# WonderfulToolchain/psxavenc

Measured on AMD Instinct MI355X. Metric: bs_v2_320x240_frames_per_sec, higher is better.
Workload: dtype int32

## Files before the change

psxavenc_amd/csrc/mdec_kernels.hip:

```cpp

#include <hip/hip_runtime.h>
#include <stdint.h>
#include <type_traits>
#include <stdlib.h>
#include <string.h>

#include "bs_vlc_lut.h"
#include "mdec_search.h"
#include "psxhip_internal.h"
#include "wave_ops.h"

namespace {

constexpr int kWavesSmall = 12, kOccSmall = 6;
constexpr int kWavesLarge = 16, kOccLarge = 4;
constexpr int kTileStride = 72;
constexpr int kZStride = 64;
constexpr int kPilotMax = 4;
constexpr int kMaxTiles = 16;
constexpr uint32_t kNoMb = 0xFFFFu;
constexpr uint32_t kRetryEmpty = 0xFFFFFFFFu, kRetryAbandoned = 0xFFFFFFFEu;
constexpr int kQueueWord = 64;
constexpr int kStartedWord = 96;
constexpr int kLeaveWord = 8;
constexpr int kLeaveWrongShift = 32, kLeaveTriedShift = 48;
constexpr unsigned kTrustCap = 63u;
constexpr float kCkMargin = 1000.0f;
constexpr int kNoTicket = 0x7FFFFFFF;
constexpr int kPilotWord = 10;
constexpr int kDistrustWord = 4;
constexpr int kQueueReservedShift = 32, kQueueHeadShift = 48;
constexpr unsigned kQueueMask = 0xFFFFu;
template <typename T>
__device__ __forceinline__ T queue_peek(T* p, int looks) {
    return looks < 4096 ? __hip_atomic_load(p, __ATOMIC_RELAXED, __HIP_MEMORY_SCOPE_AGENT) : atomicOr(p, (T)0);
}

__constant__ uint16_t c_ac_len16[BS_LUT_SIZE];
__constant__ uint32_t c_ac_code[BS_LUT_SIZE];
__constant__ uint8_t c_zagzig[64];
__constant__ uint8_t c_quant_zz[64];
__constant__ uint8_t c_dc_prefix[2][8];
// ... 11 lines not shown
    int first[kMaxBatches];
    int n_batches;
    size_t frame_stride;
    int width, height, nx, ny, nmb;
    int n_frames;
    int n_tickets;
    int uniform_max_size;
    size_t out_stride;
    int out_words;
    int out_tile;
    int max_frame_size;
    int stg_words;
    int trips;
    int it_step;
    const uint32_t* order;
    unsigned int* ticket;
    unsigned int* hint;
    unsigned int* retry;
    int retry_patience;
    int retry_cap;
    int trust_mode;
    unsigned long long* stats;
    uint32_t col_k[16];
};
typedef const BatchDesc __attribute__((address_space(4))) * BatchPtr;
typedef const int __attribute__((address_space(4))) * FirstPtr;
#define PSX_BATCHES_MANY() (((FirstPtr)(batch_table() + kMaxBatches))[kMaxBatches] > 1)
__device__ __forceinline__ BatchPtr batch_table() {
    BatchPtr p = (BatchPtr)__builtin_amdgcn_kernarg_segment_ptr();
    asm volatile("" : "+s"(p));
    return p;
}
#define PSX_JOB_INT(member) (((FirstPtr)((const char __attribute__((address_space(4)))*)batch_table() + offsetof(FrameJob, member)))[0])
__device__ __forceinline__ unsigned int* retry_slots(const FrameJob& job) {
    unsigned int* p = job.retry;
    asm volatile("" : "+s"(p));
    return p;
}
__device__ __forceinline__ unsigned long long* queue_state(const FrameJob& job) { return (unsigned long long*)&job.ticket[kQueueWord]; }
__device__ __forceinline__ unsigned draw_ticket(const FrameJob& job) { return (unsigned)atomicAdd(queue_state(job), 1ull); }
__device__ __forceinline__ unsigned long long* leave_word(const FrameJob& job) { return (unsigned long long*)&job.ticket[kLeaveWord]; }
enum {
    S_DC_BITS = 0,
    S_STG_NEXT,
    S_FOREIGN,
    S_CNT_F,
// ... 265 lines not shown

__host__ __device__ constexpr size_t lds_fixed_bytes(int waves) {
    size_t b = 0;
    b += (size_t)S_COUNT * 4;
    b += BS_LUT_SIZE * 2;
    b = (b + 3) & ~(size_t)3;
    b += BS_LUT_SIZE * 4;
    b += 32;
    b = (b + 15) & ~(size_t)15;
    b += 2 * 64 * 16 + 2 * 64;
    b += (size_t)waves * kWaveTileBytes;
    return (b + 15) & ~(size_t)15;
}
__host__ __device__ inline size_t lds_bytes(int nmb, int out_words, int stg_words, int waves) {
    size_t b = lds_fixed_bytes(waves);
    b += (size_t)out_words * 4;
    b += (size_t)stg_words * 4;
    b += (size_t)nmb * 4;
    b += (size_t)nmb * 4;
    b += (size_t)dc_chunks(nmb) * 16;
    b += (size_t)nmb * 6 * 2;
    return (b + 15) & ~(size_t)15;
}
template <int WAVES>
__device__ __forceinline__ Lds carve(char* base, int nmb, int out_words, int stg_words) {
    Lds L;
    size_t b = 0;
    L.scalars = (int*)(base + b);         b += (size_t)S_COUNT * 4;
    L.ac_len16 = (uint16_t*)(base + b);   b += BS_LUT_SIZE * 2;                    b = (b + 3) & ~(size_t)3;
    L.ac_code = (uint32_t*)(base + b);    b += BS_LUT_SIZE * 4;
    L.dc_plen = (uint8_t*)(base + b);     b += 16;
    L.dc_prefix = (uint8_t*)(base + b);   b += 16;                                 b = (b + 15) & ~(size_t)15;
    L.tab_sel = (uint4*)(base + b);       b += 64 * 16;
    L.tab_pix = (uint4*)(base + b);       b += 64 * 16;
    L.tab_nat = (uint8_t*)(base + b);     b += 64;
    L.qzz = (uint8_t*)(base + b);         b += 64;
    L.tiles = (int16_t*)(base + b);       b += (size_t)WAVES * kWaveTileBytes;     b = (b + 15) & ~(size_t)15;
    L.out = (uint32_t*)(base + b);        b += (size_t)out_words * 4;
    L.stg = (uint32_t*)(base + b);        b += (size_t)stg_words * 4;
    L.rec = (uint32_t*)(base + b);        b += (size_t)nmb * 4;
    L.mb_off = (uint32_t*)(base + b);     b += (size_t)nmb * 4;
    L.dc_fn = (int*)(base + b);           b += (size_t)dc_chunks(nmb) * 16;
    L.dcv = (int16_t*)(base + b);
    return L;
}

// ... 128 lines not shown
}
template <int CTRL>
__device__ __forceinline__ StepFn dpp_stepfn(const StepFn& f) {
    StepFn e;
    e.thr = __builtin_amdgcn_update_dpp(f.thr, f.thr, CTRL, 0xF, 0xF, false);
    e.lo = __builtin_amdgcn_update_dpp(f.lo, f.lo, CTRL, 0xF, 0xF, false);
    e.hi = __builtin_amdgcn_update_dpp(f.hi, f.hi, CTRL, 0xF, 0xF, false);
    return e;
}
__device__ __forceinline__ void scan_stepfn(StepFn& f, int lane) {
    StepFn e;
    e = dpp_stepfn<0x111>(f); if ((lane & 15) >= 1) f = compose(e, f);
    e = dpp_stepfn<0x112>(f); if ((lane & 15) >= 2) f = compose(e, f);
    e = dpp_stepfn<0x114>(f); if ((lane & 15) >= 4) f = compose(e, f);
    e = dpp_stepfn<0x118>(f); if ((lane & 15) >= 8) f = compose(e, f);
    e = dpp_stepfn<0x142>(f); if (lane & 16) f = compose(e, f);
    e = dpp_stepfn<0x143>(f); if (lane >= 32) f = compose(e, f);
}

template <int CODEC, int WAVES, int OCC, bool STATS>
__global__ __launch_bounds__(WAVES * 64, OCC) void mdec_encode_frames_kernel(const FrameJob job) {
    constexpr int kWavesPerGroup = WAVES;
    constexpr int kThreads = WAVES * 64;
    extern __shared__ __attribute__((aligned(16))) char smem[];
    const Lds L = carve<WAVES>(smem, job.nmb, job.out_words, job.stg_words);

    const int tid = (int)threadIdx.x;
    unsigned long long t_entry = 0, t_first = 0;
    if (STATS) t_entry = wall_clock64();
    const int wid = __builtin_amdgcn_readfirstlane(tid >> 6);
    const int nmb = job.nmb, nx = job.nx, ny = job.ny, W = job.width, H = job.height;
    const int nblk = nmb * 6;
    constexpr int kPilotPerWave = 2;
    const int pilot_rounds = (WAVES == kWavesLarge || nmb >= 600) ? 2 : 1;
    const int n_pilot = nmb < kWavesPerGroup * pilot_rounds ? nmb : kWavesPerGroup * pilot_rounds;

    constexpr int kLutTrips = (BS_LUT_SIZE + kThreads - 1) / kThreads;
    uint16_t lut_len[kLutTrips];
    uint32_t lut_code[kLutTrips];
#pragma unroll
    for (int j = 0; j < kLutTrips; j++) {
        const int i = tid + j * kThreads;
        lut_len[j] = i < BS_LUT_SIZE ? c_ac_len16[i] : (uint16_t)0;
        lut_code[j] = i < BS_LUT_SIZE ? c_ac_code[i] : 0u;
    }
    const uint8_t pro_plen = c_dc_plen[(tid >> 3) & 1][tid & 7], pro_prefix = c_dc_prefix[(tid >> 3) & 1][tid & 7];
// ... 350 lines not shown
                bits = wave::reduce_add(bits);
                if (lane == 0 && bits) atomicAdd(&L.scalars[S_DC_BITS], bits);
            }
            group_sync(1);
        }
        mark(1);
        const int dc_bits = CODEC == 0 ? 10 * nblk : L.scalars[S_DC_BITS];
        const int fixed_bits = dc_bits + 2 * nblk + 10;

        float cf[6];
        uint2 plo = make_uint2(0, 0), phi = make_uint2(0, 0);

        auto fetch_at = [&](uint32_t row, uint32_t col) {
            const uint4 tp = L.tab_pix[lane];
            const uint32_t o_lo = tp.x + (row << tp.z) + col, o_hi = o_lo + tp.y;
            plo = *(const uint2*)(frame + o_lo);
            phi = *(const uint2*)(frame + o_hi);
        };
        auto fetch = [&](int fx, int fy) { fetch_at((uint32_t)fy * (uint32_t)(8 * W), (uint32_t)fx * 16u); };
        auto mb_bytes = [&](const uint4& ts, uint32_t& b_lo, uint32_t& b_hi) {
            b_lo = __builtin_amdgcn_perm(plo.y, plo.x, ts.x);
            b_hi = __builtin_amdgcn_perm(phi.y, phi.x, ts.y);
        };
        auto fetch_behind = [&](uint32_t row, uint32_t col, uint32_t& b_lo, uint32_t& b_hi) {
            asm volatile("" : "+v"(b_lo), "+v"(b_hi));
            const uint4 tp = L.tab_pix[lane];
            uint32_t o_lo = tp.x + (row << tp.z) + col;
            asm volatile("" : "+v"(o_lo) : "v"(b_lo), "v"(b_hi));
            const uint32_t o_hi = o_lo + tp.y;
            plo = *(const uint2*)(frame + o_lo);
            phi = *(const uint2*)(frame + o_hi);
        };
        auto dct_mb = [&](const uint4& ts, uint32_t b_lo, uint32_t b_hi) {
            int d[8];
            u32x16 ck;
            asm volatile("s_load_dwordx16 %0, %1, %2" : "=s"(ck) : "s"(__builtin_amdgcn_kernarg_segment_ptr()), "n"(offsetof(FrameJob, col_k)));
            {
                fdct8_rows_mfma(b_lo, b_hi, make_uint2(ts.z, ts.w), d);
                const int n = lane & 31;
                int16_t* t0 = tileT + (n >> 3) * kTileStride + (n & 7) + (lane >> 5) * 32;
                store_row_outputs(t0, d);
                if (n < 16) store_row_outputs(t0 + 4 * kTileStride, d + 4);
            }
            wave_sync();
            if (lane < 48) {
                uint4 q;
                asm volatile("ds_read2_b64 %0, %2 offset1:1\n\ts_waitcnt lgkmcnt(0)"
                             : "=v"(q), "+s"(ck) : "v"((uint32_t)(uintptr_t)&tileT[blk * kTileStride + r8 * 8]) : "memory");
                fdct8_col_acc_k(q.x, q.y, __builtin_amdgcn_alignbit(q.w, q.w, 16), __builtin_amdgcn_alignbit(q.z, q.z, 16), ck, d);
                if (r8 == 0) d[0] = CODEC == 0 ? (int)((uint32_t)quant_dc(d[0] >> 17) << 17) : 0;
                uint4 o;
                o.x = pack_sh17(d[1], d[0]);
                o.y = pack_sh17(d[3], d[2]);
                o.z = pack_sh17(d[5], d[4]);
                o.w = pack_sh17(d[7], d[6]);
                *(uint4*)&tileZ[lane * 8] = o;
            }
            wave_sync();
        };

        if (tid == 0) {
            int hint = L.scalars[S_HINT];
// ... 28 lines not shown
                const int sh = L.scalars[S_SHARED_HINT];
                if ((sh >> 8) == max_size) h0 = sh & 0xFF;
            }
            L.scalars[S_PILOT_HI] = h0;
        }
        auto search_reset = [&](MdecSearch& st) {
            mdec_search_init(st);
            st.best = in_loop(st.best);
            {
                const int z = in_loop(0);
                st.lo = z; st.staged = z; st.pad = z;
                st.fail = (uint64_t)(uint32_t)z | ((uint64_t)(uint32_t)in_loop(0) << 32);
                st.fs[0] = st.fs[1] = st.fb[0] = st.fb[1] = z;
                st.gs[0] = st.gs[1] = st.gb[0] = st.gb[1] = z;
            }
        };
        unsigned long long trace = 0;
        int n_pass = 0, first_abort = 0, guess0 = 0;
        int guess;
        MdecSearch* srch = (MdecSearch*)&L.scalars[S_SEARCH];
        group_sync(1);
        if (L.scalars[S_PILOT_GUESS] == 0) {
        float cfp[kPilotPerWave][6];
#pragma unroll
        for (int i = 0; i < kPilotPerWave; i++) {
            const int pi = wid + i * kWavesPerGroup;
            if (pi < n_pilot) {
                const unsigned u = (unsigned)(2 * pi + 1);
                const int p_fy = (int)((u * (unsigned)ny) / (unsigned)(2 * n_pilot));
                const int p_fx = (int)((((u * 40503u) >> 1) & 0xFFFFu) * (unsigned)nx >> 16);
                fetch(n_pilot == nmb ? pi % nx : p_fx, n_pilot == nmb ? pi / nx : p_fy);
                {
                    const uint4 ts = L.tab_sel[lane];
                    uint32_t b_lo, b_hi;
                    mb_bytes(ts, b_lo, b_hi);
                    dct_mb(ts, b_lo, b_hi);
                }
#pragma unroll
                for (int b = 0; b < 6; b++) cf[b] = lane == 0 ? 0.0f : (float)(int)tileZ[b * kZStride + lc.zsrc];
                wave_sync();
            }
#pragma unroll
            for (int b = 0; b < 6; b++) cfp[i][b] = pi < n_pilot ? cf[b] : 0.0f;
        }
        if (tid == 0) {
            L.scalars[S_PILOTED] = 1;
            const int h0 = L.scalars[S_PILOT_HI];
            MdecSearch st;
            search_reset(st);
            *srch = st;
            const MdecPilot pl = mdec_pilot_next(st, h0, limit_bits, fixed_bits, 0);
            L.scalars[S_PILOT_N] = pl.n;
            L.scalars[S_PILOT_SCALE0 + 0] = pl.s[0];
            L.scalars[S_PILOT_SCALE0 + 1] = pl.s[1];
            L.scalars[S_PILOT_SCALE0 + 2] = pl.s[2];
            L.scalars[S_PILOT_LO] = in_loop(0);
        }
        for (;;) {
            group_sync(1);
            const int np = L.scalars[S_PILOT_N];
            if (np == 0) break;
            if (wid < n_pilot) {
                for (int j = 0; j < np; j++) {
                    const int s = L.scalars[S_PILOT_SCALE0 + j];
                    const QuantK k = make_quant(lc.quant, s);
                    int acc = 0;
#pragma unroll
                    for (int i = 0; i < kPilotPerWave; i++)
                        if (i < pilot_rounds) acc += count_mb(cfp[i], k, lc, L.ac_len16) & 0xFF;
                    const int t = wave::reduce_add(acc);
                    if (lane == 0) atomicAdd(&L.scalars[S_PILOT_BITS0 + j], t);
                }
            }
            group_sync(1);
            if (tid == 0) {
                MdecSearch st = *srch;
                for (int j = 0; j < np; j++) {
                    const int s = L.scalars[S_PILOT_SCALE0 + j];
                    const int est = (int)((long long)L.scalars[S_PILOT_BITS0 + j] * nmb / n_pilot) + fixed_bits;
                    mdec_search_note(st, s, est, est, limit_bits);
                    L.scalars[S_PILOT_BITS0 + j] = 0;
                }
                *srch = st;
                const int round = L.scalars[S_PILOT_LO] + 1;
                const MdecPilot pl = mdec_pilot_next(st, L.scalars[S_PILOT_HI], limit_bits, fixed_bits, round);
// ... 38 lines not shown
                if (tid == 0) L.scalars[S_STG_NEXT] = 0;
                group_sync(5);
            }
            typedef const char __attribute__((address_space(4))) * OrderBytes;
            typedef const uint32_t __attribute__((address_space(4))) * OrderPtr;
            const OrderBytes order_b = (OrderBytes)(uintptr_t)job.order;
            const int n_tickets = job.trips * kWavesPerGroup;
            auto order_at = [&](int t) -> uint2 {
                const uint32_t byte = min((uint32_t)t, (uint32_t)n_tickets) * 8u;
                const OrderPtr e = (OrderPtr)(order_b + byte);
                return make_uint2(e[0], e[1]);
            };
            int cur_t = wid, nxt_t = wid + kWavesPerGroup;
            uint2 cur_o = order_at(cur_t);
            uint2 nxt_o = order_at(nxt_t);
            fetch_at(cur_o.x & 0x7FFFFFFFu, cur_o.y & 0xFFFFu);
            const QuantK kc = make_quant(lc.quant, count_scale ? count_scale : 1);
            const QuantK ke = make_quant(lc.quant, emit_scale ? emit_scale : 1);
            int acc_cnt = 0;
            int acc_edef = 0;
            int n_codes = 0;
            int emit_bits = 0, mb_done = 0;
            int prev_len = 0;
            const uint32_t thr_low = (uint32_t)((lc.quant * (count_scale ? count_scale : 1) + 1) >> 1);
            const uint32_t thr_emit = (uint32_t)((lc.quant * (emit_scale ? emit_scale : 1) + 1) >> 1);
            const uint32_t thr_list = count_scale ? thr_low : thr_emit;
            const uint32_t low_off = thr_list - 1u, low_span = lane == 0 ? 0u : 2u * thr_list - 1u;
            const uint32_t emit_off = thr_emit - 1u, emit_span = lane == 0 ? 0u : 2u * thr_emit - 1u;
            auto flush = [&]() {
                if (count_scale) {
                    const int tf = wave::reduce_add(acc_cnt & 0xFFFF), td = wave::reduce_add((int)((unsigned)acc_cnt >> 16));
                    if (lane == 0) { atomicAdd(&L.scalars[S_CNT_F], tf); atomicAdd(&L.scalars[S_CNT_D], td); }
                    acc_cnt = 0;
                }
                if (emit_scale) {
                    const int td = wave::reduce_add(acc_edef), tc = n_codes;
                    if (lane == 0) {
                        atomicAdd(&L.scalars[S_EMIT_BITS], emit_bits);
                        atomicAdd(&L.scalars[S_EMIT_D], td);
                        atomicAdd(&L.scalars[S_NNZ], tc - 6 * mb_done);
                    }
                    acc_edef = 0; n_codes = 0; emit_bits = 0;
                }
                if (lane == 0) atomicAdd(&L.scalars[S_CK_DONE], mb_done);
                mb_done = 0;
            };
            const int check_t = (job.trips >= 8 && L.scalars[S_ABORTS_LEFT] > 0) ? (job.trips >> 2) * kWavesPerGroup : n_tickets;
            bool aborted = false, checked = false;

            for (int it = 0; cur_t < n_tickets; it++) {
                if (!checked && cur_t >= check_t) {
                    checked = true;
                    flush();
                    int arrived = 0;
                    if (lane == 0) arrived = atomicAdd(&L.scalars[S_CK_WAVES], 1);
                    const bool judge = __builtin_amdgcn_readfirstlane(arrived) == kWavesPerGroup - 1;
                    unsigned ck_s1 = 0, ck_sq = 0;
                    bool records_ok = false;
                    if (judge && emit_scale) records_ok = __hip_atomic_load(&L.scalars[S_STG_NEXT], __ATOMIC_RELAXED, __HIP_MEMORY_SCOPE_WORKGROUP) <= job.stg_words;
                    if (records_ok) {
                        for (int t = lane; t < check_t; t += 64) {
                            const OrderPtr oe = (OrderPtr)(order_b + (uint32_t)t * 8u);
                            if ((int)oe[0] < 0) {
                                const unsigned x = *(const uint32_t*)((const char*)L.rec + (oe[1] >> 16)) >> 18;
                                ck_s1 += x;
                                ck_sq += x * x;
                            }
                        }
                        ck_s1 = (unsigned)wave::reduce_add((int)ck_s1);
                        ck_sq = (unsigned)wave::reduce_add((int)ck_sq);
                    }
                    if (judge && lane == 0) {
                        const int done = L.scalars[S_CK_DONE];
                        long long pa = 0, pb = 0;
                        if (count_scale) pa = (long long)L.scalars[S_CNT_F] * nmb / done + fixed_bits;
                        if (emit_scale) pb = (long long)L.scalars[S_EMIT_BITS] * nmb / done + 10;
                        int margin = (limit_bits - fixed_bits) / 50;
                        if (emit_scale && records_ok && done > 1 && done < nmb) {
                            const float n = (float)done, mean = (float)ck_s1 / n;
                            float var = (float)ck_sq / n - mean * mean;
                            var = var > 0.0f ? var : 0.0f;
                            const float se = 4.0f * __builtin_sqrtf(var * n * (1.0f - n / (float)nmb)) * ((float)nmb / n);
                            margin = (int)(se * kCkMargin * 0.001f);
                        }
// ... 2 lines not shown
                            const int cur = emit_scale ? emit_scale : count_scale + 1, far = cur > 8 ? cur >> 2 : 2;
                            if (g && L.scalars[S_PILOTED] && (g - cur >= far || cur - g >= far)) {
                                const bool too_low = emit_scale && pb > (long long)limit_bits + 4 * margin;
                                const bool too_high = count_scale && pa <= (long long)limit_bits - 4 * margin;
                                if (!too_low && !too_high) g = 0;
                            }
                        }
                        if (g) {
                            L.scalars[S_ABORT] = g | (n_pass << 8);
                            L.scalars[S_ABORTS_LEFT] = L.scalars[S_ABORTS_LEFT] - 1;
                            atomicMax(&L.scalars[S_MB_NEXT], 0x40000000);
                        }
                    }
                }
                if (WAVES == kWavesSmall) {
                    asm volatile("s_bitcmp1_b32 %0, %1\n\ts_cbranch_scc1 1f\n\ts_setprio 0\n\ts_branch 2f\n1:\ts_setprio 1\n2:" : : "s"(prio_bits4), "s"(it) : "scc");
                }
                int drawn = 0;
                if (lane == 0) drawn = atomicAdd(&L.scalars[S_MB_NEXT], 1);
                const bool valid = (int)cur_o.x < 0;
                const uint32_t rec_byte = cur_o.y >> 16;
                const int mbe = (int)(rec_byte >> 2);
                {
                    const uint4 ts = L.tab_sel[lane];
                    uint32_t b_lo, b_hi;
                    mb_bytes(ts, b_lo, b_hi);
                    fetch_behind(nxt_o.x & 0x7FFFFFFFu, nxt_o.y & 0xFFFFu, b_lo, b_hi);
                    if (valid) dct_mb(ts, b_lo, b_hi);
                }
                cur_t = nxt_t;
                cur_o = nxt_o;
                nxt_t = __builtin_amdgcn_readfirstlane(drawn);
                nxt_o = order_at(nxt_t);
                if (!valid) continue;
                mb_done++;

                int ci[6];
#pragma unroll
                for (int b = 0; b < 6; b++) ci[b] = (int)tileZ[b * kZStride + lc.zsrc];
                wave_sync();

                if (!emit_scale) {
                    float cff[6];
#pragma unroll
                    for (int b = 0; b < 6; b++) cff[b] = lane == 0 ? 0.0f : (float)ci[b];
                    const int a = count_mb(cff, kc, lc, L.ac_len16);
                    acc_cnt += (a & 0xFF) | ((a >> 8) << 16);
                    continue;
                }
                constexpr std::true_type yes{};
// ... 131 lines not shown
                                len = i != 0 ? 12 : 10;
                            }
                        } else {
                            const uint64_t dcmask = dcm;
                            if (is_dc) {
                                const int bi = bcarry + wave::popc_below(dcmask);
                                dc_code<CODEC>((int)L.dcv[mbe * 6 + bi], bi >= 2, L.dc_plen, L.dc_prefix, len, code);
                                if (bi > 0) {
                                    code |= 2u << len;
                                    len += 2;
                                }
                            }
                            if (!single) bcarry += (int)__builtin_popcountll(dcmask);
                        }
                        {
                            const int add = is_last ? 2 : 0;
                            code = (code << add) | (uint32_t)add;
                            len += add;
                        }
                    };
                    bool have_room = true;
                    auto stage_alloc = [&](uint32_t mb_bits) -> uint32_t {
                        const int ndw = (int)((mb_bits + 31u) >> 5);
                        int off = 0;
                        if (lane == 0) {
                            off = atomicAdd(&L.scalars[S_STG_NEXT], ndw);
                            *(uint32_t*)((char*)L.rec + rec_byte) = (uint32_t)off | (mb_bits << 16);
                        }
                        off = __builtin_amdgcn_readfirstlane(off);
                        have_room = off + ndw <= job.stg_words;
                        emit_bits += (int)mb_bits;
                        return (uint32_t)off;
                    };
                    auto put_codes = [&](uint32_t base_dw, uint32_t bit, int len, uint32_t code) {
                        if (have_room) {
                            if (len) put_bits_lds(L.stg, base_dw, bit, len, code);
                        }
                    };
                    bool low = cs && !dense;
                    if (low && count > 64) {
                        int sc = 0, kcarry = 0;
                        for (int base = 0; base < count; base += 64) {
                            const int i = base + lane;
                            const bool live = i < count;
                            uint32_t e = clist[i];
                            e = live ? e : (63u << 17);
                            const int k = (int)__builtin_amdgcn_ubfe(e, 17, 6);
                            const bool is_dc = k == 0;
                            const bool is_ac = live && !is_dc;
                            float magf;
                            asm("v_cvt_f32_i32_sdwa %0, sext(%1) dst_sel:DWORD dst_unused:UNUSED_PAD src0_sel:WORD_0" : "=v"(magf) : "v"(e));
                            QuantK ck, ek;
                            ck.inv = __builtin_bit_cast(float, __builtin_amdgcn_ds_bpermute(k << 2, __builtin_bit_cast(int, kc.inv)));
                            ck.bias = __builtin_fmaf(0.25f, ck.inv, 0.5f);
// ... 16 lines not shown
                        wave_sync();
                        count = sc;
                        low = false;
                    }
                    if (count <= 64) {
                        int len, deficit, cnt16, nc;
                        uint32_t code;
                        if (low) chunk(yes, yes, yes, 0, len, code, deficit, cnt16, nc);
                        else chunk(no, no, yes, 0, len, code, deficit, cnt16, nc);
                        const int incl = wave::inclusive_scan_add(len);
                        const uint32_t base_dw = stage_alloc((uint32_t)__builtin_amdgcn_readlane(incl, 63));
                        put_codes(base_dw, (uint32_t)(incl - len), len, code);
                        acc_edef += deficit;
                        acc_cnt += cnt16;
                        n_codes += nc;
                    } else {
                        int lsum = 0;
                        for (int base = 0; base < count; base += 64) {
                            int len, deficit, cnt16, nc;
                            uint32_t code;
                            chunk(no, no, no, base, len, code, deficit, cnt16, nc);
                            lsum += len;
                        }
                        const uint32_t base_dw = stage_alloc((uint32_t)wave::reduce_add(lsum));
                        uint32_t pos = 0;
                        kcarry_a = 0;
                        kcarry_b = 0;
                        bcarry = 0;
                        for (int base = 0; base < count; base += 64) {
                            int len, deficit, cnt16, nc;
                            uint32_t code;
                            chunk(no, no, no, base, len, code, deficit, cnt16, nc);
                            const int incl = wave::inclusive_scan_add(len);
                            put_codes(base_dw, pos + (uint32_t)(incl - len), len, code);
                            pos += (uint32_t)__builtin_amdgcn_readlane(incl, 63);
                            acc_edef += deficit;
                            n_codes += nc;
                        }
                    }
                    wave_sync();
                };
                if (count_scale) emit_mb(yes);
                else emit_mb(no);
            }
            if (WAVES == kWavesSmall) __builtin_amdgcn_s_setprio(2);
            flush();
            group_sync(3);
// ... 351 lines not shown

namespace {
__global__ __launch_bounds__(256) void mdec_stage_in_kernel(const uint4* src, uint4* dst, int n16) {
    const int i = (int)(blockIdx.x * 256 + threadIdx.x);
    if (i < n16) dst[i] = src[i];
}
}
extern "C" hipError_t psxhip_mdec_stage_in_launch(const void* src_mapped, void* d_dst, size_t bytes, void* stream) {
    const int n16 = (int)(bytes >> 4);
    if (n16 <= 0) return hipSuccess;
    hipLaunchKernelGGL(mdec_stage_in_kernel, dim3((unsigned)((n16 + 255) / 256)), dim3(256), 0, (hipStream_t)stream, (const uint4*)src_mapped,
                       (uint4*)d_dst, n16);
    return hipGetLastError();
}

#include "mdec_split.inc"

extern "C" hipError_t psxhip_mdec_fdct_launch(const int16_t* d_in, int16_t* d_out, int n_blocks, void* stream) {
    if (n_blocks <= 0) return hipSuccess;
    hipLaunchKernelGGL(mdec_fdct_probe_kernel, dim3((unsigned)((n_blocks + 5) / 6)), dim3(64), 0, (hipStream_t)stream, d_in, d_out, n_blocks);
    return hipGetLastError();
}

extern "C" size_t psxhip_mdec_lds_bytes(int nmb, int out_words, int stg_words, int large) {
    return lds_bytes(nmb, out_words, stg_words, large ? kWavesLarge : kWavesSmall);
}
extern "C" int psxhip_mdec_threads_per_group(int large) { return (large ? kWavesLarge : kWavesSmall) * 64; }

extern "C" hipError_t psxhip_mdec_upload_tables(void) {
    hipError_t e;
    if ((e = hipMemcpyToSymbol(HIP_SYMBOL(c_ac_len16), bs_ac_len16_lut, sizeof(bs_ac_len16_lut))) != hipSuccess) return e;
    if ((e = hipMemcpyToSymbol(HIP_SYMBOL(c_ac_code), bs_ac_code_lut, sizeof(bs_ac_code_lut))) != hipSuccess) return e;
    if ((e = hipMemcpyToSymbol(HIP_SYMBOL(c_zagzig), bs_zagzig, sizeof(bs_zagzig))) != hipSuccess) return e;
    if ((e = hipMemcpyToSymbol(HIP_SYMBOL(c_quant_zz), bs_quant_zz, sizeof(bs_quant_zz))) != hipSuccess) return e;
    uint8_t pre[2][8], pl[2][8];
    for (int i = 0; i < 8; i++) {
        pre[0][i] = bs_dc_chroma_prefix[i]; pl[0][i] = bs_dc_chroma_plen[i];
        pre[1][i] = bs_dc_luma_prefix[i];   pl[1][i] = bs_dc_luma_plen[i];
    }
    if ((e = hipMemcpyToSymbol(HIP_SYMBOL(c_dc_prefix), pre, sizeof(pre))) != hipSuccess) return e;
    if ((e = hipMemcpyToSymbol(HIP_SYMBOL(c_dc_plen), pl, sizeof(pl))) != hipSuccess) return e;
    return hipSuccess;
}

static int pick_it_step(int trips) {
    if (trips <= 2) return 1;
    const int want = (trips * 382 + 500) / 1000;
    for (int d = 0; d < trips; d++) {
        const int cand[2] = {want + d, want - d};
// ... 59 lines not shown
    for (int i = 0, first = 0; i < a->n_batches && i < kMaxBatches; i++) {
        job.batch[i].frames = a->batches[i].d_frames;
        job.batch[i].out = a->batches[i].d_out;
        job.batch[i].results = a->batches[i].d_results;
        job.batch[i].max_sizes = a->batches[i].d_frame_max_sizes;
        job.first[i] = first;
        first += a->batches[i].n_frames;
    }
    for (int i = a->n_batches; i < kMaxBatches; i++) job.first[i] = 0x7FFFFFFF;
    job.frame_stride = a->frame_stride;
    job.width = a->width;
    job.height = a->height;
    job.nx = a->width / 16;
    job.ny = a->height / 16;
    job.nmb = job.nx * job.ny;
    job.n_frames = a->n_frames;
    job.n_tickets = a->n_tickets;
    job.uniform_max_size = a->uniform_max_size;
    job.out_stride = a->out_stride;
    job.out_words = a->out_words;
    job.out_tile = a->out_tile;
    job.max_frame_size = a->max_frame_size;
    job.stg_words = a->stg_words;
    job.ticket = a->d_ticket;
    job.hint = a->d_hint;
    job.retry = a->d_retry;
    job.retry_cap = a->retry_cap;
    job.retry_patience = a->retry_patience;
    job.stats = a->d_stats;
    job.trust_mode = a->trust_mode;
    { constexpr ColCoeffs ck = col_coeffs(); for (int i = 0; i < 16; i++) job.col_k[i] = ck.k[i]; }
    job.trips = (job.nmb + waves_ - 1) / waves_;
    job.it_step = pick_it_step(job.trips);
    job.order = a->d_order;
    const int waves = waves_;
    const size_t lds = lds_bytes(job.nmb, job.out_words, job.stg_words, waves);
    const dim3 grid((unsigned)a->grid), block((unsigned)waves * 64u);
    hipStream_t st = (hipStream_t)a->stream;
#define PSX_LAUNCH(CODEC)                                                                                             \
    do {                                                                                                              \
        if (job.stats) {                                                                                              \
            if (a->large) hipLaunchKernelGGL((mdec_encode_frames_kernel<CODEC, kWavesLarge, kOccLarge, true>), grid, block, lds, st, job); \
            else hipLaunchKernelGGL((mdec_encode_frames_kernel<CODEC, kWavesSmall, kOccSmall, true>), grid, block, lds, st, job);          \
        } else {                                                                                                      \
            if (a->large) hipLaunchKernelGGL((mdec_encode_frames_kernel<CODEC, kWavesLarge, kOccLarge, false>), grid, block, lds, st, job); \
            else hipLaunchKernelGGL((mdec_encode_frames_kernel<CODEC, kWavesSmall, kOccSmall, false>), grid, block, lds, st, job);          \
        }                                                                                                             \
    } while (0)
    switch (a->codec) {
    case 0: PSX_LAUNCH(0); break;
    case 1: PSX_LAUNCH(1); break;
    default: PSX_LAUNCH(2); break;
    }
#undef PSX_LAUNCH
    return hipGetLastError();
}

extern "C" hipError_t psxhip_mdec_set_max_lds(int codec, size_t bytes) {
    hipError_t e = hipSuccess;
// ... 23 lines not shown
```

psxavenc_amd/csrc/psxhip_api.cpp:

```cpp
#include <hip/hip_runtime.h>

#include <climits>
#include <cstdarg>
#include <cstdio>
#include <cstdlib>
#include <cstring>
#include <dlfcn.h>
#include <ctime>
#include <mutex>
#include <thread>
#include <vector>

#include "device_buffer.h"
#include "psxhip_internal.h"

namespace {

thread_local char g_err[512] = "";
std::mutex g_tables_mu;
struct SplitGate {
    std::mutex mu;
    hipEvent_t last = nullptr;
    hipStream_t last_stream = nullptr;
    bool pending = false;
// ... 22 lines not shown
extern "C" void psxhip_set_error(const char* fmt, ...) {
    va_list ap;
    va_start(ap, fmt);
    vsnprintf(g_err, sizeof g_err, fmt, ap);
    va_end(ap);
}

extern "C" const char* psxhip_last_error(void) { return g_err; }
extern "C" const char* psxhip_version(void) { return "psxav_hip 0.4 (gfx950, " PSXHIP_MDEC_KERNEL_REV ")"; }

extern "C" int psxhip_device_count(void) {
    int n = 0;
    if (hipGetDeviceCount(&n) != hipSuccess) return 0;
    return n;
}

int psxhip_ensure_device(int device) { return ensure_device(device); }


constexpr int kLanes = 2;
struct psxhip_mdec_ctx {
    int device, codec, width, height, nmb;
    int max_frame_size, out_words, stg_words;
    int groups_max;
    int large;
    size_t lds_bytes;
    unsigned int* d_ticket;
    unsigned int* d_retry;
    int retry_cap;
    int lanes, next_lane;
    hipStream_t lane_stream[2];
    hipEvent_t lane_in[2], lane_done[2];
    bool lane_pending[2];
    int retry_patience;
    int trust_mode;
    unsigned long long* d_stats;
    uint32_t* d_order;
    uint32_t* d_order_large;
    int n_cu;
    hipStream_t stream;
    uint8_t* d_frames[2];
    uint8_t* d_out[2];
    psxhip_mdec_result_t* d_res[2];
    int32_t* d_sizes[2];
    uint8_t* h_in[2];
    uint8_t* h_out[2];
// ... 1 lines not shown
    hipStream_t stream2;
    int cap_frames;
    size_t cap_out_stride;
    uint8_t* h_call;
    uint8_t* d_call;
    uint8_t* d_call_frame;
    size_t call_out_off, call_res_off;
    bool call_disabled;
    bool call_no_flush;
    volatile uint32_t* hdp_flush;
    bool call_bar;
    int call_hint;
    unsigned call_seq;
    unsigned char* d_split_ws;
    size_t split_ws_stride;
    int split_max;
    unsigned long long split_patience;
    int wh_frame, wh_seg, wh_launches, wh_residue;
    long long split_launches;
};

namespace {
int mdec_geometry(int width, int height, int max_frame_size, size_t lds_cu, int* large, int* out_words, int* stg_words,
                  size_t* lds_bytes) {
    const int nmb = (width / 16) * (height / 16);
    const int image = (max_frame_size + 3) / 4;
    const int sw = image + nmb + 2;
    if (sw > 0xFFFF) return 0;
    const int tiles[4] = {image, 2048, 1024, 512};
    int lg = 1, ow = 0;
    for (int shape = 0; shape < 2 && !ow; shape++) {
        for (int i = 0; i < 4 && !ow; i++) {
            const int t = tiles[i] < image ? tiles[i] : image;
            if ((image + t - 1) / t > 16) continue;
            if ((shape ? 1 : 2) * psxhip_mdec_lds_bytes(nmb, t + 2, sw, shape) <= lds_cu) {
                lg = shape;
                ow = t + 2;
            }
        }
    }
    if (!ow) {
        lg = 1;
        ow = (image < 512 ? image : 512) + 2;
    }
    const size_t need = psxhip_mdec_lds_bytes(nmb, ow, sw, lg);
    if (large) *large = lg;
    if (out_words) *out_words = ow;
    if (stg_words) *stg_words = sw;
    if (lds_bytes) *lds_bytes = need;
    return need <= lds_cu;
}
bool mdec_args_ok(int codec, int width, int height, int max_frame_size) {
    return !(codec < 0 || codec > 2 || width <= 0 || height <= 0 || (width % 16) || (height % 16) || width > 1024 ||
             height > 1024 || max_frame_size < 8);
}
}

extern "C" int psxhip_mdec_query_geometry(int device, int codec, int width, int height, int max_frame_size,
                                          psxhip_mdec_geometry_t* out) {
    if (out) memset(out, 0, sizeof(*out));
    if (!mdec_args_ok(codec, width, height, max_frame_size)) {
        psxhip_set_error("bad MDEC geometry: codec %d, %dx%d, budget %d", codec, width, height, max_frame_size);
        return PSXHIP_EINVAL;
    }
    int rc = ensure_device(device);
    if (rc) return rc;
    hipDeviceProp_t prop;
    HIP_TRY(hipGetDeviceProperties(&prop, device), PSXHIP_EDEVICE);
// ... 26 lines not shown
    *out = nullptr;
    if (!mdec_args_ok(codec, width, height, max_frame_size)) {
        psxhip_set_error("bad MDEC geometry: codec %d, %dx%d, budget %d", codec, width, height, max_frame_size);
        return PSXHIP_EINVAL;
    }
    int rc = ensure_device(device);
    if (rc) return rc;

    psxhip_mdec_ctx* c = (psxhip_mdec_ctx*)calloc(1, sizeof(*c));
    if (!c) return PSXHIP_ENOMEM;
    struct Guard {
        psxhip_mdec_ctx* p;
        ~Guard() { if (p) psxhip_mdec_destroy(p); }
    } guard{c};
    c->device = device;
    c->codec = codec;
    c->width = width;
    c->height = height;
    c->nmb = (width / 16) * (height / 16);
    c->max_frame_size = max_frame_size;
    hipDeviceProp_t prop;
    HIP_TRY(hipGetDeviceProperties(&prop, device), PSXHIP_EDEVICE);
    const size_t lds_cu = (size_t)prop.maxSharedMemoryPerMultiProcessor;
    if (!mdec_geometry(width, height, max_frame_size, lds_cu, &c->large, &c->out_words, &c->stg_words, &c->lds_bytes)) {
        psxhip_set_error("frame budget %d with %d macroblocks needs %zu B of LDS (> %zu); see psxhip_mdec_query_geometry",
                         max_frame_size, c->nmb, c->lds_bytes, lds_cu);
        return PSXHIP_EINVAL;
    }
    HIP_TRY(psxhip_mdec_set_max_lds(codec, lds_cu), PSXHIP_EDEVICE);
    c->groups_max = prop.multiProcessorCount * (c->large ? 1 : 2);
    if (c->groups_max > 1040) c->groups_max = 1040;
    if (const char* e = getenv("PSXHIP_MDEC_TRUST")) c->trust_mode = atoi(e);

    c->lanes = 1;
    HIP_TRY(hipMalloc((void**)&c->d_ticket, kLanes * 128 * sizeof(unsigned int)), PSXHIP_ENOMEM);
    HIP_TRY(hipMemset(c->d_ticket, 0, kLanes * 128 * sizeof(unsigned int)), PSXHIP_EDEVICE);
    if (!getenv("PSXHIP_MDEC_NO_RETRY_QUEUE")) {
        c->retry_cap = 1 << 16;
        c->retry_patience = 256;
        if (const char* e = getenv("PSXHIP_MDEC_QUEUE_PATIENCE")) c->retry_patience = atoi(e);
        HIP_TRY(hipMalloc((void**)&c->d_retry, (size_t)kLanes * c->retry_cap * sizeof(unsigned int)), PSXHIP_ENOMEM);
        HIP_TRY(hipMemset(c->d_retry, 0xFF, (size_t)kLanes * c->retry_cap * sizeof(unsigned int)), PSXHIP_EDEVICE);
    }
    c->n_cu = prop.multiProcessorCount;
    c->call_no_flush = getenv("PSXHIP_NO_HDP_FLUSH") != nullptr;
    {
        c->split_max = 12;
// ... 1 lines not shown
        if (c->split_max > 64) c->split_max = 64;
        if (const char* e = getenv("PSXHIP_MDEC_SPLIT_PATIENCE")) c->split_patience = strtoull(e, nullptr, 10);
        if (const char* e = getenv("PSXHIP_MDEC_SPLIT_WITHHOLD")) {
            char seg[16] = {0};
            int fr = 0, launches = 1, residue = 0;
            const int n = sscanf(e, "%d:%15[^:]:%d:%d", &fr, seg, &launches, &residue);
            if (n >= 2 && fr >= 0 && launches > 0) {
                c->wh_frame = fr;
                c->wh_seg = strcmp(seg, "mid") == 0 ? INT_MIN : atoi(seg);
                c->wh_launches = launches;
                c->wh_residue = residue != 0;
            }
        }
        psxhip_mdec_split_geo_t g;
        if (c->split_max > 0 && psxhip_mdec_split_geometry(codec, width, height, max_frame_size, 1, c->n_cu, &g)) {
            c->split_ws_stride = g.ws_stride;
            const size_t bytes = (size_t)(kLanes + 1) * c->split_max * g.ws_stride;
            HIP_TRY(hipMalloc((void**)&c->d_split_ws, bytes), PSXHIP_ENOMEM);
            HIP_TRY(hipMemset(c->d_split_ws, 0, bytes), PSXHIP_EDEVICE);
        } else {
            c->split_max = 0;
        }
    }
    const bool both = !c->large && psxhip_mdec_lds_bytes(c->nmb, c->out_words, c->stg_words, 1) <= lds_cu;
    for (int shape = c->large; shape <= (both ? 1 : c->large); shape++) {
        const int n = psxhip_mdec_pass_table(width, height, shape, nullptr, 0);
        const size_t tab_bytes = ((size_t)n + 1) * 2 * sizeof(uint32_t);
        uint32_t* h = (uint32_t*)malloc(tab_bytes);
        if (!h) { psxhip_set_error("out of host memory"); return PSXHIP_ENOMEM; }
        if (psxhip_mdec_pass_table(width, height, shape, h, n + 1) != n) { free(h); psxhip_set_error("out of host memory"); return PSXHIP_ENOMEM; }
        uint32_t** dst = shape == c->large ? &c->d_order : &c->d_order_large;
        hipError_t e = hipMalloc((void**)dst, tab_bytes);
        if (e == hipSuccess) e = hipMemcpy(*dst, h, tab_bytes, hipMemcpyHostToDevice);
        free(h);
        if (e != hipSuccess) { psxhip_set_error("pass order table: %s", hipGetErrorString(e)); return PSXHIP_ENOMEM; }
    }
    if (const char* e = getenv("PSXHIP_MDEC_STATS")) {
        if (atoi(e)) {
            HIP_TRY(hipMalloc((void**)&c->d_stats, PSXHIP_MDEC_STATS_TOTAL * sizeof(unsigned long long)), PSXHIP_ENOMEM);
            HIP_TRY(hipMemset(c->d_stats, 0, PSXHIP_MDEC_STATS_TOTAL * sizeof(unsigned long long)), PSXHIP_EDEVICE);
        }
    }
    HIP_TRY(hipStreamSynchronize(nullptr), PSXHIP_EDEVICE);
    guard.p = nullptr;
    *out = c;
    return PSXHIP_OK;
}
// ... 73 lines not shown
            }
            HIP_TRY(psxhip_mdec_split_launch(&sp), PSXHIP_EDEVICE);
            gate.last_stream = stream;
            gate.pending = true;
            if (d_done_flag && gate_hold) *gate_hold = std::move(lk);
            return PSXHIP_OK;
        }
    }
    const bool small_batch = c->d_order_large && n_frames <= c->n_cu;
    psxhip_mdec_launch_t a;
    a.batches = batches;
    a.n_batches = nb;
    a.frame_stride = frame_stride;
    a.width = c->width;
    a.height = c->height;
    a.codec = c->codec;
    a.n_frames = n_frames;
    a.uniform_max_size = uniform_max_size;
    a.out_stride = out_stride;
    a.out_words = c->out_words;
    a.out_tile = c->out_words - 2;
    a.max_frame_size = c->max_frame_size;
    a.stg_words = c->stg_words;
    a.n_tickets = n_frames;
    a.grid = a.n_tickets < c->groups_max ? a.n_tickets : c->groups_max;
    a.large = c->large || small_batch;
    a.stream = stream;
    a.d_ticket = c->d_ticket + 128 * lane;
    a.d_hint = c->d_ticket + 2;
    const bool queue = c->d_retry && n_frames > a.grid && n_frames <= 8 * a.grid && n_frames < c->retry_cap;
    a.d_retry = queue ? c->d_retry + (size_t)lane * c->retry_cap : nullptr;
    a.retry_cap = queue ? c->retry_cap : 0;
    a.retry_patience = c->retry_patience;
    a.d_order = small_batch ? c->d_order_large : c->d_order;
    a.d_stats = c->d_stats;
    a.trust_mode = c->trust_mode;
    HIP_TRY(psxhip_mdec_launch(&a), PSXHIP_EDEVICE);
    return PSXHIP_OK;
}

static int mdec_ensure_lanes(psxhip_mdec_ctx* c) {
    for (int l = 0; l < kLanes; l++) {
        if (!c->lane_stream[l]) HIP_TRY(hipStreamCreateWithFlags(&c->lane_stream[l], hipStreamNonBlocking), PSXHIP_EDEVICE);
        if (!c->lane_in[l]) HIP_TRY(hipEventCreateWithFlags(&c->lane_in[l], hipEventDisableTiming), PSXHIP_EDEVICE);
        if (!c->lane_done[l]) HIP_TRY(hipEventCreateWithFlags(&c->lane_done[l], hipEventDisableTiming), PSXHIP_EDEVICE);
    }
// ... 477 lines not shown
```

psxavenc_amd/csrc/psxhip_internal.h:

```cpp
#pragma once
#include <hip/hip_runtime.h>
#include <stddef.h>
#include <stdint.h>

#include "../../include/psxav_hip.h"

#define PSXHIP_MDEC_KERNEL_REV "mdec-k3.8"
#define PSXHIP_ADPCM_KERNEL_REV "adpcm-k5.4"

#ifdef __cplusplus
extern "C" {
#endif

typedef struct {
	const psxhip_mdec_batch_t *batches;
	int n_batches;
	size_t frame_stride;
	int width, height, codec;
	int n_frames;
	int n_tickets;
	int uniform_max_size;
	size_t out_stride;
	int out_words;
	int out_tile;
	int max_frame_size;
	int stg_words;
	int grid;
	int large;
	void *stream;
	unsigned int *d_ticket;
	unsigned int *d_hint;
	unsigned int *d_retry;
	int retry_cap;
	int retry_patience;
	unsigned long long *d_stats;
	int trust_mode;
	const uint32_t *d_order;
} psxhip_mdec_launch_t;

typedef struct {
	int seg_mbs, segs;
	int img_words;
	size_t ws_stride, ws_slots, ws_dcq, ws_img, ws_done;
	size_t lds_bytes;
} psxhip_mdec_split_geo_t;
typedef struct {
	const uint8_t *d_frames;
	uint8_t *d_out;
	psxhip_mdec_result_t *d_results;
	const int32_t *d_frame_max_sizes;
	size_t frame_stride, out_stride;
	int width, height, codec, n_frames, uniform_max_size, max_frame_size;
	psxhip_mdec_split_geo_t geo;
	void *d_ws;
	unsigned int *d_lost;
	unsigned int *d_done_flag;
	unsigned int done_seq;
	int hint;
	void *stream;
	unsigned long long patience;
	int wh_frame, wh_seg, wh_residue;
} psxhip_mdec_split_t;
int psxhip_mdec_split_geometry(int codec, int width, int height, int max_frame_size, int n_frames, int n_cu, psxhip_mdec_split_geo_t *g);
hipError_t psxhip_mdec_split_launch(const psxhip_mdec_split_t *a);
int psxhip_mdec_encode_batches_frame_kernel(psxhip_mdec_ctx_t *ctx, const psxhip_mdec_batch_t *batches, int n_batches,
                                            size_t frame_stride, int uniform_max_size, size_t out_stride, void *stream);

size_t psxhip_mdec_lds_bytes(int nmb, int out_words, int stg_words, int large);
int psxhip_mdec_threads_per_group(int large);
hipError_t psxhip_mdec_upload_tables(void);
hipError_t psxhip_mdec_set_max_lds(int codec, size_t bytes);
int psxhip_mdec_pass_order(int width, int height, int large, uint32_t *out, int cap);
int psxhip_mdec_pass_table(int width, int height, int large, uint32_t *out , int cap);
hipError_t psxhip_mdec_launch(const psxhip_mdec_launch_t *a);
hipError_t psxhip_mdec_stage_in_launch(const void *src_mapped, void *d_dst, size_t bytes, void *stream);
hipError_t psxhip_mdec_fdct_launch(const int16_t *d_in, int16_t *d_out, int n_blocks, void *stream);

int psxhip_mdec_encode_frames_host_rows(psxhip_mdec_ctx_t *ctx, const uint8_t *frames, int n_frames,
                                        const int32_t *frame_max_sizes, int uniform_max_size, uint8_t *out,
                                        size_t out_stride, psxhip_mdec_result_t *results, int row_bytes);
int psxhip_xa_encode_streams_host_flags(int device, int format, int stereo, int frequency, int bits, int file_number,
                                        int channel_number, const int16_t *samples, int n_streams, int64_t stream_stride,
                                        int samples_per_stream, const int32_t *lbas, psxhip_adpcm_state_t *states,
                                        uint8_t *out, int64_t out_stride, int finalize, const uint8_t *eof_flags);

int psxhip_xa_assemble_scatter(int device, const uint8_t *d_units, int n_sectors, int format, int stereo, int frequency, int bits,
                               int file_number, int channel_number, int first_lba, const uint8_t *d_eof_flags, uint32_t eof_bits,
                               uint8_t *d_out, const int32_t *d_dst_sector, int n_streams, size_t units_stream_stride,
                               size_t out_stream_stride, void *stream);
void psxhip_adpcm_pick_chunking(long long total_units, int rows, int device, int *chunk_units, int *warmup_units);
int psxhip_adpcm_chunked_threshold(int n_chains);
// ... 71 lines not shown
```

Measured before the change: 8.668 million.

## Give each wave a private LDS staging piece to avoid atomic stage allocation

Adds per-wave private staging pieces of 256 dwords in extra LDS, used by the small-wave kernel when two workgroups still fit per CU. Macroblock bitstream allocation bumps a wave-local pointer and records the offset directly, instead of doing an LDS atomicAdd on a shared counter for every macroblock, falling back to the shared allocator when a piece is full. It also hoists the tab_pix load into the loop body, makes the abort check re-armable, and adds scalar hints. The costs are more LDS per group and a zero-fill of each piece when emit_scale is set.

```diff
diff --git a/psxavenc_amd/csrc/mdec_kernels.hip b/psxavenc_amd/csrc/mdec_kernels.hip
--- a/psxavenc_amd/csrc/mdec_kernels.hip
+++ b/psxavenc_amd/csrc/mdec_kernels.hip
@@ -18,6 +18,7 @@
 constexpr int kZStride = 64;
 constexpr int kPilotMax = 4;
 constexpr int kMaxTiles = 16;
+constexpr int kStagePiece = PSXHIP_MDEC_STAGE_PIECE;
 constexpr uint32_t kNoMb = 0xFFFFu;
 constexpr uint32_t kRetryEmpty = 0xFFFFFFFFu, kRetryAbandoned = 0xFFFFFFFEu;
 constexpr int kQueueWord = 64;
@@ -75,6 +76,7 @@
     int trust_mode;
     unsigned long long* stats;
     uint32_t col_k[16];
+    int stg_first;
 };
 typedef const BatchDesc __attribute__((address_space(4))) * BatchPtr;
 typedef const int __attribute__((address_space(4))) * FirstPtr;
@@ -386,6 +388,14 @@
     b += (size_t)nmb * 6 * 2;
     return (b + 15) & ~(size_t)15;
 }
+__host__ __device__ inline size_t stg_byte_offset(int out_words) { return lds_fixed_bytes(kWavesSmall) + (size_t)out_words * 4; }
+__host__ __device__ inline int piece_first(int nmb, int out_words, int stg_words) {
+    const size_t span = (lds_bytes(nmb, out_words, stg_words, kWavesSmall) - stg_byte_offset(out_words)) / 4;
+    return (int)((span + kStagePiece - 1) / kStagePiece * kStagePiece);
+}
+__host__ __device__ inline size_t piece_bytes(int nmb, int out_words, int stg_words) {
+    return stg_byte_offset(out_words) + ((size_t)piece_first(nmb, out_words, stg_words) + (size_t)kWavesSmall * kStagePiece) * 4 - lds_bytes(nmb, out_words, stg_words, kWavesSmall);
+}
 template <int WAVES>
 __device__ __forceinline__ Lds carve(char* base, int nmb, int out_words, int stg_words) {
     Lds L;
@@ -560,6 +570,7 @@
 __global__ __launch_bounds__(WAVES * 64, OCC) void mdec_encode_frames_kernel(const FrameJob job) {
     constexpr int kWavesPerGroup = WAVES;
     constexpr int kThreads = WAVES * 64;
+    constexpr bool kPieces = WAVES == kWavesSmall;
     extern __shared__ __attribute__((aligned(16))) char smem[];
     const Lds L = carve<WAVES>(smem, job.nmb, job.out_words, job.stg_words);
 
@@ -956,9 +967,8 @@
             b_lo = __builtin_amdgcn_perm(plo.y, plo.x, ts.x);
             b_hi = __builtin_amdgcn_perm(phi.y, phi.x, ts.y);
         };
-        auto fetch_behind = [&](uint32_t row, uint32_t col, uint32_t& b_lo, uint32_t& b_hi) {
+        auto fetch_behind = [&](const uint4& tp, uint32_t row, uint32_t col, uint32_t& b_lo, uint32_t& b_hi) {
             asm volatile("" : "+v"(b_lo), "+v"(b_hi));
-            const uint4 tp = L.tab_pix[lane];
             uint32_t o_lo = tp.x + (row << tp.z) + col;
             asm volatile("" : "+v"(o_lo) : "v"(b_lo), "v"(b_hi));
             const uint32_t o_hi = o_lo + tp.y;
@@ -971,7 +981,7 @@
             asm volatile("s_load_dwordx16 %0, %1, %2" : "=s"(ck) : "s"(__builtin_amdgcn_kernarg_segment_ptr()), "n"(offsetof(FrameJob, col_k)));
             {
                 fdct8_rows_mfma(b_lo, b_hi, make_uint2(ts.z, ts.w), d);
-                const int n = lane & 31;
+                const int n = in_loop(lane) & 31;
                 int16_t* t0 = tileT + (n >> 3) * kTileStride + (n & 7) + (lane >> 5) * 32;
                 store_row_outputs(t0, d);
                 if (n < 16) store_row_outputs(t0 + 4 * kTileStride, d + 4);
@@ -1046,10 +1056,12 @@
         group_sync(1);
         if (L.scalars[S_PILOT_GUESS] == 0) {
         float cfp[kPilotPerWave][6];
+        int n_pilot_f = n_pilot;
+        asm volatile("" : "+s"(n_pilot_f));
 #pragma unroll
         for (int i = 0; i < kPilotPerWave; i++) {
             const int pi = wid + i * kWavesPerGroup;
-            if (pi < n_pilot) {
+            if (pi < n_pilot_f) {
                 const unsigned u = (unsigned)(2 * pi + 1);
                 const int p_fy = (int)((u * (unsigned)ny) / (unsigned)(2 * n_pilot));
                 const int p_fx = (int)((((u * 40503u) >> 1) & 0xFFFFu) * (unsigned)nx >> 16);
@@ -1065,7 +1077,7 @@
                 wave_sync();
             }
 #pragma unroll
-            for (int b = 0; b < 6; b++) cfp[i][b] = pi < n_pilot ? cf[b] : 0.0f;
+            for (int b = 0; b < 6; b++) cfp[i][b] = pi < n_pilot_f ? cf[b] : 0.0f;
         }
         if (tid == 0) {
             L.scalars[S_PILOTED] = 1;
@@ -1084,7 +1096,7 @@
             group_sync(1);
             const int np = L.scalars[S_PILOT_N];
             if (np == 0) break;
-            if (wid < n_pilot) {
+            if (wid < n_pilot_f) {
                 for (int j = 0; j < np; j++) {
                     const int s = L.scalars[S_PILOT_SCALE0 + j];
                     const QuantK k = make_quant(lc.quant, s);
@@ -1169,6 +1181,16 @@
             int n_codes = 0;
             int emit_bits = 0, mb_done = 0;
             int prev_len = 0;
+            int piece_next = kStagePiece - 1;
+            if (kPieces) {
+                const int first = PSX_JOB_INT(stg_first);
+                if (first) {
+                    piece_next = first + wid * kStagePiece;
+                    if (emit_scale)
+#pragma unroll
+                        for (int j = 0; j < kStagePiece / 64; j++) L.stg[piece_next + j * 64 + lane] = 0u;
+                }
+            }
             const uint32_t thr_low = (uint32_t)((lc.quant * (count_scale ? count_scale : 1) + 1) >> 1);
             const uint32_t thr_emit = (uint32_t)((lc.quant * (emit_scale ? emit_scale : 1) + 1) >> 1);
             const uint32_t thr_list = count_scale ? thr_low : thr_emit;
@@ -1192,12 +1214,13 @@
                 if (lane == 0) atomicAdd(&L.scalars[S_CK_DONE], mb_done);
                 mb_done = 0;
             };
-            const int check_t = (job.trips >= 8 && L.scalars[S_ABORTS_LEFT] > 0) ? (job.trips >> 2) * kWavesPerGroup : n_tickets;
-            bool aborted = false, checked = false;
+            int check_t = (job.trips >= 8 && L.scalars[S_ABORTS_LEFT] > 0) ? (job.trips >> 2) * kWavesPerGroup : n_tickets;
+            bool aborted = false;
 
             for (int it = 0; cur_t < n_tickets; it++) {
-                if (!checked && cur_t >= check_t) {
-                    checked = true;
+                if (cur_t >= check_t) {
+                    const int check_n = check_t;
+                    check_t = 0x7FFFFFFF;
                     flush();
                     int arrived = 0;
                     if (lane == 0) arrived = atomicAdd(&L.scalars[S_CK_WAVES], 1);
@@ -1206,7 +1229,7 @@
                     bool records_ok = false;
                     if (judge && emit_scale) records_ok = __hip_atomic_load(&L.scalars[S_STG_NEXT], __ATOMIC_RELAXED, __HIP_MEMORY_SCOPE_WORKGROUP) <= job.stg_words;
                     if (records_ok) {
-                        for (int t = lane; t < check_t; t += 64) {
+                        for (int t = lane; t < check_n; t += 64) {
                             const OrderPtr oe = (OrderPtr)(order_b + (uint32_t)t * 8u);
                             if ((int)oe[0] < 0) {
                                 const unsigned x = *(const uint32_t*)((const char*)L.rec + (oe[1] >> 16)) >> 18;
@@ -1255,10 +1278,12 @@
                 const uint32_t rec_byte = cur_o.y >> 16;
                 const int mbe = (int)(rec_byte >> 2);
                 {
-                    const uint4 ts = L.tab_sel[lane];
+                    uint4 ts = L.tab_sel[lane];
+                    uint4 tp = L.tab_pix[lane];
+                    asm volatile("" : "+v"(ts.x), "+v"(ts.y), "+v"(tp.x));
                     uint32_t b_lo, b_hi;
                     mb_bytes(ts, b_lo, b_hi);
-                    fetch_behind(nxt_o.x & 0x7FFFFFFFu, nxt_o.y & 0xFFFFu, b_lo, b_hi);
+                    fetch_behind(tp, nxt_o.x & 0x7FFFFFFFu, nxt_o.y & 0xFFFFu, b_lo, b_hi);
                     if (valid) dct_mb(ts, b_lo, b_hi);
                 }
                 cur_t = nxt_t;
@@ -1436,6 +1461,13 @@
                     bool have_room = true;
                     auto stage_alloc = [&](uint32_t mb_bits) -> uint32_t {
                         const int ndw = (int)((mb_bits + 31u) >> 5);
+                        emit_bits += (int)mb_bits;
+                        if (kPieces && __builtin_expect((piece_next & (kStagePiece - 1)) + ndw < kStagePiece, 1)) {
+                            const int off = piece_next;
+                            piece_next += ndw;
+                            if (lane == 0) *(uint32_t*)((char*)L.rec + rec_byte) = (uint32_t)off | (mb_bits << 16);
+                            return (uint32_t)off;
+                        }
                         int off = 0;
                         if (lane == 0) {
                             off = atomicAdd(&L.scalars[S_STG_NEXT], ndw);
@@ -1443,7 +1475,6 @@
                         }
                         off = __builtin_amdgcn_readfirstlane(off);
                         have_room = off + ndw <= job.stg_words;
-                        emit_bits += (int)mb_bits;
                         return (uint32_t)off;
                     };
                     auto put_codes = [&](uint32_t base_dw, uint32_t bit, int len, uint32_t code) {
@@ -1506,7 +1537,7 @@
                             chunk(no, no, no, base, len, code, deficit, cnt16, nc);
                             lsum += len;
                         }
-                        const uint32_t base_dw = stage_alloc((uint32_t)wave::reduce_add(lsum));
+                        const uint32_t base_dw = stage_alloc((uint32_t)__builtin_amdgcn_readfirstlane(wave::reduce_add(lsum)));
                         uint32_t pos = 0;
                         kcarry_a = 0;
                         kcarry_b = 0;
@@ -1904,9 +1935,10 @@
     return hipGetLastError();
 }
 
-extern "C" size_t psxhip_mdec_lds_bytes(int nmb, int out_words, int stg_words, int large) {
-    return lds_bytes(nmb, out_words, stg_words, large ? kWavesLarge : kWavesSmall);
-}
+extern "C" size_t psxhip_mdec_lds_bytes(int nmb, int out_words, int stg_words, int large, int pieces) {
+    return lds_bytes(nmb, out_words, stg_words, large ? kWavesLarge : kWavesSmall) + (pieces && !large ? piece_bytes(nmb, out_words, stg_words) : 0);
+}
+extern "C" int psxhip_mdec_stage_first(int nmb, int out_words, int stg_words) { return piece_first(nmb, out_words, stg_words); }
 extern "C" int psxhip_mdec_threads_per_group(int large) { return (large ? kWavesLarge : kWavesSmall) * 64; }
 
 extern "C" hipError_t psxhip_mdec_upload_tables(void) {
@@ -2012,6 +2044,7 @@
     job.out_tile = a->out_tile;
     job.max_frame_size = a->max_frame_size;
     job.stg_words = a->stg_words;
+    job.stg_first = a->large ? 0 : a->stg_first;
     job.ticket = a->d_ticket;
     job.hint = a->d_hint;
     job.retry = a->d_retry;
@@ -2024,7 +2057,7 @@
     job.it_step = pick_it_step(job.trips);
     job.order = a->d_order;
     const int waves = waves_;
-    const size_t lds = lds_bytes(job.nmb, job.out_words, job.stg_words, waves);
+    const size_t lds = lds_bytes(job.nmb, job.out_words, job.stg_words, waves) + (job.stg_first ? piece_bytes(job.nmb, job.out_words, job.stg_words) : 0);
     const dim3 grid((unsigned)a->grid), block((unsigned)waves * 64u);
     hipStream_t st = (hipStream_t)a->stream;
 #define PSX_LAUNCH(CODEC)                                                                                             \
diff --git a/psxavenc_amd/csrc/psxhip_api.cpp b/psxavenc_amd/csrc/psxhip_api.cpp
--- a/psxavenc_amd/csrc/psxhip_api.cpp
+++ b/psxavenc_amd/csrc/psxhip_api.cpp
@@ -68,6 +68,7 @@
 struct psxhip_mdec_ctx {
     int device, codec, width, height, nmb;
     int max_frame_size, out_words, stg_words;
+    int stg_first;
     int groups_max;
     int large;
     size_t lds_bytes;
@@ -115,7 +116,7 @@
 
 namespace {
 int mdec_geometry(int width, int height, int max_frame_size, size_t lds_cu, int* large, int* out_words, int* stg_words,
-                  size_t* lds_bytes) {
+                  size_t* lds_bytes, int* stg_first = nullptr) {
     const int nmb = (width / 16) * (height / 16);
     const int image = (max_frame_size + 3) / 4;
     const int sw = image + nmb + 2;
@@ -126,7 +127,7 @@
         for (int i = 0; i < 4 && !ow; i++) {
             const int t = tiles[i] < image ? tiles[i] : image;
             if ((image + t - 1) / t > 16) continue;
-            if ((shape ? 1 : 2) * psxhip_mdec_lds_bytes(nmb, t + 2, sw, shape) <= lds_cu) {
+            if ((shape ? 1 : 2) * psxhip_mdec_lds_bytes(nmb, t + 2, sw, shape, 0) <= lds_cu) {
                 lg = shape;
                 ow = t + 2;
             }
@@ -136,7 +137,9 @@
         lg = 1;
         ow = (image < 512 ? image : 512) + 2;
     }
-    const size_t need = psxhip_mdec_lds_bytes(nmb, ow, sw, lg);
+    const bool pieces = !lg && 2 * psxhip_mdec_lds_bytes(nmb, ow, sw, 0, 1) <= lds_cu;
+    const size_t need = psxhip_mdec_lds_bytes(nmb, ow, sw, lg, pieces);
+    if (stg_first) *stg_first = pieces ? psxhip_mdec_stage_first(nmb, ow, sw) : 0;
     if (large) *large = lg;
     if (out_words) *out_words = ow;
     if (stg_words) *stg_words = sw;
@@ -209,7 +212,7 @@
     hipDeviceProp_t prop;
     HIP_TRY(hipGetDeviceProperties(&prop, device), PSXHIP_EDEVICE);
     const size_t lds_cu = (size_t)prop.maxSharedMemoryPerMultiProcessor;
-    if (!mdec_geometry(width, height, max_frame_size, lds_cu, &c->large, &c->out_words, &c->stg_words, &c->lds_bytes)) {
+    if (!mdec_geometry(width, height, max_frame_size, lds_cu, &c->large, &c->out_words, &c->stg_words, &c->lds_bytes, &c->stg_first)) {
         psxhip_set_error("frame budget %d with %d macroblocks needs %zu B of LDS (> %zu); see psxhip_mdec_query_geometry",
                          max_frame_size, c->nmb, c->lds_bytes, lds_cu);
         return PSXHIP_EINVAL;
@@ -257,7 +260,7 @@
             c->split_max = 0;
         }
     }
-    const bool both = !c->large && psxhip_mdec_lds_bytes(c->nmb, c->out_words, c->stg_words, 1) <= lds_cu;
+    const bool both = !c->large && psxhip_mdec_lds_bytes(c->nmb, c->out_words, c->stg_words, 1, 0) <= lds_cu;
     for (int shape = c->large; shape <= (both ? 1 : c->large); shape++) {
         const int n = psxhip_mdec_pass_table(width, height, shape, nullptr, 0);
         const size_t tab_bytes = ((size_t)n + 1) * 2 * sizeof(uint32_t);
@@ -377,6 +380,7 @@
     a.out_tile = c->out_words - 2;
     a.max_frame_size = c->max_frame_size;
     a.stg_words = c->stg_words;
+    a.stg_first = c->stg_first;
     a.n_tickets = n_frames;
     a.grid = a.n_tickets < c->groups_max ? a.n_tickets : c->groups_max;
     a.large = c->large || small_batch;
diff --git a/psxavenc_amd/csrc/psxhip_internal.h b/psxavenc_amd/csrc/psxhip_internal.h
--- a/psxavenc_amd/csrc/psxhip_internal.h
+++ b/psxavenc_amd/csrc/psxhip_internal.h
@@ -5,7 +5,8 @@
 
 #include "../../include/psxav_hip.h"
 
-#define PSXHIP_MDEC_KERNEL_REV "mdec-k3.8"
+#define PSXHIP_MDEC_KERNEL_REV "mdec-k3.9"
+#define PSXHIP_MDEC_STAGE_PIECE 256
 #define PSXHIP_ADPCM_KERNEL_REV "adpcm-k5.4"
 
 #ifdef __cplusplus
@@ -25,6 +26,7 @@
 	int out_tile;
 	int max_frame_size;
 	int stg_words;
+	int stg_first;
 	int grid;
 	int large;
 	void *stream;
@@ -66,7 +68,8 @@
 int psxhip_mdec_encode_batches_frame_kernel(psxhip_mdec_ctx_t *ctx, const psxhip_mdec_batch_t *batches, int n_batches,
                                             size_t frame_stride, int uniform_max_size, size_t out_stride, void *stream);
 
-size_t psxhip_mdec_lds_bytes(int nmb, int out_words, int stg_words, int large);
+size_t psxhip_mdec_lds_bytes(int nmb, int out_words, int stg_words, int large, int pieces);
+int psxhip_mdec_stage_first(int nmb, int out_words, int stg_words);
 int psxhip_mdec_threads_per_group(int large);
 hipError_t psxhip_mdec_upload_tables(void);
 hipError_t psxhip_mdec_set_max_lds(int codec, size_t bytes);
```

After: 8.541 million. 0.985x the previous value.
